# rhuangr/MARL-Maze

Measured on AMD Instinct MI355X. Metric: env-steps/sec (2-agent 10x10 maze) + PPO updates/sec, higher is better.
Workload: dtype f32; 1 GPU; PPO rollout+GAE+update over 65536 parallel 10x10 2-agent mazes per GPU (configs[2], the north-star workload: 65,536 parallel 10x10 mazes per GPU); mazes_per_gpu=65536, maze=10x10 (layout 19x19), horizon=16, global_batch=1048575, minibatch=209715, minibatch_steps_per_iter=25, parallelism=dp1, rollout=stream launches, gemm=x2, parity_mode=True

## Files before the change

### include/marlmaze.h

```cpp
#ifndef MARLMAZE_H
#define MARLMAZE_H

#include <stdint.h>

#ifdef __cplusplus
extern "C" {
#endif

#define MM_OBS_DIM 65
#define MM_MASK_DIM 6
#define MM_RNG_WORDS 625
#define MM_MAX_SIDE 41
#define MM_MAZES_PER_BLOCK 32

#define MM_E_ARG (-1)
#define MM_E_SIZE (-2)

#define MM_ST_GEN_FAIL 1u
#define MM_ST_BAD_MOVE 2u

typedef struct {
    int8_t x, y, dir, flags;
    int8_t lmx, lmy, olsx, olsy;
    int8_t minx, maxx, miny, maxy;
// ... 149 lines not shown
              const uint16_t* w1, const float* b1, int N1, const uint16_t* w2, const float* b2, int N2, float* out,
              int ldc, void* stream);
int mm_trunk3_head_sample_ok(int prec, int M, int K0, int N0, int N1, int N2, int lda);
int mm_trunk3_head_sample(int prec, const float* h0, int lda, int M, int K0, const uint16_t* w0, const float* b0,
                          int N0, const uint16_t* w1, const float* b1, int N1, const uint16_t* w2, const float* b2,
                          int N2, const float* head_w, const float* head_b, const uint8_t* masks, uint64_t seed,
                          uint64_t offset, const uint64_t* offset_dev, int8_t* actions, float* logp,
                          float* joint_logp, float* logits, float* h3, int ldh3, void* stream);

int mm_ppo_loss_partials(int M);
int mm_ppo_loss(const float* heads, const uint8_t* masks, const int8_t* actions, const float* old_logp,
                const float* adv, int M, float clip, float* coef, float* partial, void* stream);
int mm_ppo_loss_bwd(const float* heads, const uint8_t* masks, const int8_t* actions, const float* coef,
                    const float* dloss, int M, float* dheads, void* stream);

int mm_colsum(const float* x, long R, int N, float* part, int G, float* out, void* stream);
typedef struct {
    const float* x;
    long R;
    int N;
    float* out;
} mm_colsum_seg_t;
typedef struct {
    const float* x;
    long n;
    int S;
    float* out;
} mm_wsum_seg_t;
long mm_colsum_multi_ws_len(const mm_colsum_seg_t* segs, int nseg);
int mm_colsum_multi(const mm_colsum_seg_t* segs, int nseg, float* ws, void* stream);
// ... 136 lines not shown
```

### marl-maze_amd/csrc/policy_device.h

```cpp
#pragma once
#include <hip/hip_runtime.h>
#include <math.h>
#include <stdint.h>

#include "marlmaze.h"

namespace mm {

__device__ __forceinline__ uint4 philox(uint4 c, uint2 k) {
#pragma unroll
    for (int r = 0; r < 10; r++) {
        const uint32_t lo0 = 0xD2511F53u * c.x, hi0 = __umulhi(0xD2511F53u, c.x);
        const uint32_t lo1 = 0xCD9E8D57u * c.z, hi1 = __umulhi(0xCD9E8D57u, c.z);
        c = make_uint4(hi1 ^ c.y ^ k.x, lo1, hi0 ^ c.w ^ k.y, lo0);
        k.x += 0x9E3779B9u;
        k.y += 0xBB67AE85u;
    }
    return c;
}

__device__ __forceinline__ float u01(uint32_t x) { return (float)(x >> 8) * (1.0f / 16777216.0f); }

template <int MODE>
__device__ __forceinline__ float act_row(const float ml[5], float kl, const uint8_t* __restrict__ mk, int row,
// ... 98 lines not shown
        if constexpr (MODE == MM_ACT_SAMPLE) offset += offset_dev ? *offset_dev : 0ull;
        lp = act_row<MODE>(l, kl, masks + (size_t)row * MM_MASK_DIM, row, seed, offset, move, mark);
        act[2 * row] = (int8_t)move;
        act[2 * row + 1] = (int8_t)mark;
        if (logp) logp[row] = lp;
        if (logits) {
#pragma unroll
            for (int o = 0; o < 5; o++) logits[(size_t)row * 6 + o] = l[o];
            logits[(size_t)row * 6 + 5] = kl;
        }
    }
    const float other = __shfl_down(lp, kHeadLanes);
    if (joint && lead && (row & 1) == 0) joint[row >> 1] = lp + (row + 1 < M ? other : 0.f);
}

}
```

### marl-maze_amd/csrc/rl_kernels.hip

```cpp
#include <hip/hip_runtime.h>
#include <math.h>
#include <stdint.h>

#include <algorithm>

#include "marlmaze.h"
#include "policy_device.h"

namespace mm {

struct GaeArgs {
    const float* rew;
    const float* val;
    const uint8_t* done;
    const float* lv;
    int T, N;
    float g, gl;
    float* adv;
    float* rtg;
};

__device__ __forceinline__ float gae_delta(float r, float v, bool d, bool have_next, float v_next, bool d_next,
                                           float g) {
    if (d || !have_next) return __fsub_rn(r, v);
// ... 230 lines not shown
                                    __uint_as_float(v[3]));
            }
        }
#pragma unroll
        for (int s = 0; s < NS; s++) heads_fma4(hv[s], W + 4 * j + 32 * s, kSpan, acc);
    } else if (row < M) {
        heads_row_dot(h + (size_t)row * ldh, K, W, kSpan, j, acc);
    }
    heads_butterfly(acc);
    float v = acc[0];
#pragma unroll
    for (int o = 1; o < 6; o++) v = j == o ? acc[o] : v;
    if (row < M && j < 6) logits[(size_t)row * 6 + j] = v + b[j];
}

__device__ __forceinline__ float row_logp(const float* z, const uint8_t* mk, int move, int mark, float* grad) {
    float mx = -INFINITY;
#pragma unroll
    for (int j = 0; j < 5; j++)
        if (mk[j]) mx = fmaxf(mx, z[j]);
    float se = 0.f;
    float e[5];
#pragma unroll
    for (int j = 0; j < 5; j++) {
        e[j] = mk[j] ? expf(z[j] - mx) : 0.f;
        se += e[j];
    }
    const float lse = logf(se);
    const float lpm = mk[move] ? (z[move] - mx) - lse : -INFINITY;
    const float k = mk[5] ? z[5] : -INFINITY;
    const float p = 1.f / (1.f + expf(-k));
    const float pm = mark ? p : 1.f - p;
    if (grad) {
        const float inv = 1.f / se;
#pragma unroll
        for (int j = 0; j < 5; j++) grad[j] = mk[j] ? ((j == move ? 1.f : 0.f) - e[j] * inv) : 0.f;
        grad[5] = mk[5] ? (mark ? 1.f - p : -p) : 0.f;
    }
    return lpm + logf(pm);
}

constexpr int kLossThreads = 256;

__global__ __launch_bounds__(kLossThreads) void k_ppo_loss(const float* __restrict__ z, const uint8_t* __restrict__ mk,
                                                           const int8_t* __restrict__ act,
                                                           const float* __restrict__ old_lp,
                                                           const float* __restrict__ adv, int M, float clip,
                                                           float* __restrict__ coef, float* __restrict__ partial) {
    __shared__ float red[kLossThreads];
    const int i = blockIdx.x * kLossThreads + threadIdx.x;
    float term = 0.f;
    if (i < M) {
        float lp = 0.f;
#pragma unroll
        for (int a = 0; a < 2; a++) {
            const int r = 2 * i + a;
            lp += row_logp(z + (size_t)r * 6, mk + (size_t)r * 6, act[2 * r], act[2 * r + 1], nullptr);
        }
        const float ratio = expf(lp - old_lp[i]);
        const float A = adv[i];
        const float s1 = ratio * A;
        const float rc = fminf(fmaxf(ratio, 1.f - clip), 1.f + clip);
        const float s2 = rc * A;
        term = fminf(s1, s2);
        const bool inside = ratio >= 1.f - clip && ratio <= 1.f + clip;
        float dd;
        if (s1 < s2) dd = A;
        else if (s1 > s2) dd = inside ? A : 0.f;
        else dd = 0.5f * A + (inside ? 0.5f * A : 0.f);
        coef[i] = -dd * ratio / (float)M;
    }
    red[threadIdx.x] = term;
    __syncthreads();
    for (int w = kLossThreads / 2; w > 0; w >>= 1) {
        if (threadIdx.x < w) red[threadIdx.x] += red[threadIdx.x + w];
        __syncthreads();
    }
    if (threadIdx.x == 0) partial[blockIdx.x] = red[0];
}

__global__ __launch_bounds__(256) void k_ppo_loss_bwd(const float* __restrict__ z, const uint8_t* __restrict__ mk,
                                                      const int8_t* __restrict__ act, const float* __restrict__ coef,
                                                      const float* __restrict__ dloss, int M,
                                                      float* __restrict__ dz) {
    const int r = blockIdx.x * blockDim.x + threadIdx.x;
    if (r >= 2 * M) return;
    float g[6];
    row_logp(z + (size_t)r * 6, mk + (size_t)r * 6, act[2 * r], act[2 * r + 1], g);
    const float c = coef[r >> 1] * dloss[0];
#pragma unroll
    for (int j = 0; j < 6; j++) dz[(size_t)r * 6 + j] = c * g[j];
}
// ... 258 lines not shown
```

### marl-maze_amd/csrc/x3mlp.hip

```cpp
#include <hip/hip_runtime.h>
#include <stdint.h>
#include <stdlib.h>

#include <algorithm>
#include <type_traits>

#include "marlmaze.h"
#include "policy_device.h"

namespace mm {
namespace x3 {

typedef __attribute__((ext_vector_type(8))) short bf16x8;
typedef __attribute__((ext_vector_type(4))) float f32x4;
typedef __attribute__((ext_vector_type(8))) _Float16 f16x8;

enum { P_X3 = MM_PREC_X3, P_F16 = MM_PREC_F16, P_X2 = MM_PREC_X2 };
template <int P>
struct Prec {
    static constexpr int kPlanes = P == P_X3 ? 3 : P == P_X2 ? 2 : 1;
    static constexpr int kBlk = 512 * kPlanes;
    static constexpr bool kScaled = P != P_X3;
};
constexpr float kX2Lo = 2048.f;
// ... 1803 lines not shown
            const int row = 16 * tn + 4 * (lane >> 4) + g;
            if (row < N && col < K) out[(size_t)row * K + col] = v[g] * cscale;
        }
    };
#pragma unroll
    for (int r = 0; r < RN; r++)
#pragma unroll
        for (int tk = 0; tk < NTK; tk++) put(acc[r * NTK + tk], RN * wave + r, tk);
#pragma unroll
    for (int e = 0; e < EX; e++) {
        const int j = wave + kWgWaves * e;
        if (j < kRem) put(acc[RN * NTK + e], kWgWaves * RN + j / NTK, j % NTK);
    }
}

constexpr int tr_pitch(int T) {
    int w = 4 * T;
    while (w % 16 != 4) w++;
    return w;
}

template <int TN, int NTK>
__global__ __launch_bounds__(kWgThreads) void k_wgrad_tr(const uint32_t* __restrict__ dy, int lddy,
                                                         const uint32_t* __restrict__ x, int ldx, int M, int N, int K,
                                                         int rows, int nslices, int ncb, float cscale,
                                                         float* __restrict__ ws) {
    constexpr int P = P_X2;
    constexpr int RN = TN / kWgWaves;
    constexpr int kRem = (TN - kWgWaves * RN) * NTK;
    constexpr int EX = (kRem + kWgWaves - 1) / kWgWaves;
// ... 1722 lines not shown
}

extern "C" int mm_gemm_wgrad_slices(int prec, int M, int N, int K) {
    if (M <= 0 || N <= 0 || K <= 0 || (prec != MM_PREC_X3 && prec != MM_PREC_F16 && prec != MM_PREC_X2))
        return MM_E_ARG;
    const WgPlan p = wg_plan(prec, M, N, K);
    return p.TPW ? p.nslices : MM_E_ARG;
}

extern "C" int mm_gemm_wgrad_partials(int prec, const float* dy, int lddy, float dscale, const float* x, int ldx, int M,
                                      int N, int K, float cscale, float* ws, void* stream) {
    if (M <= 0) return MM_E_ARG;
    return gemm_wgrad(prec, dy, lddy, dscale, x, ldx, M, N, K, cscale, ws, nullptr, stream);
}

extern "C" int mm_critic_update_ok(int M, int K0, int ldx) {
    if (M <= 0 || K0 <= 128 || K0 > 132 || (K0 & 1) || (ldx & 1) || ldx < K0) return 0;
    const size_t wmax = std::max(ldx, 64);
    if ((size_t)(M + 320) * wmax * 4 >= ((size_t)1 << 31)) return 0;
    if (!bres_enabled()) return 0;
    BresPlan pl;
    int cfg = C_PAIR;
    return bres_plan(MM_PREC_X2, M, 64, K0, ldx, 64, true, pl, cfg) && bres_plan(MM_PREC_X2, M, 64, 64, 64, 64, true, pl, cfg) &&
                   bres_plan(MM_PREC_X2, M, 1, 64, 64, 1, false, pl, cfg)
               ? 1
               : 0;
}

extern "C" int mm_critic_update(const float* x, int ldx, int K0, int M, const float* rtg, const uint16_t* w0_tp,
                                const float* b0, const uint16_t* w1_tp, const uint16_t* w1t_tp, const float* b1,
// ... 25 lines not shown
```

### marl-maze_amd/marlmaze/PPO.py

```python
import math
import os
import random
import warnings

import numpy as np
import torch

from . import _lib, networks, ops, rollout, update, x3
from .dist import DP
from .networks import Actor, Critic

MODEL_PATH = "PPO.pth"
CRITIC_STREAM = os.environ.get("MARLMAZE_CRITIC_STREAM", "on")
CRITIC_STREAM_MAX_SAMPLES = int(os.environ.get("MARLMAZE_CRITIC_STREAM_MAX", "65536"))


def _ppo_loss_fwd(heads, mk, a8, old_logp, adv, clip):
    L = _lib.lib()
    M = old_logp.shape[0]
    old_logp, adv = old_logp.contiguous(), adv.contiguous()
    coef = torch.empty(M, dtype=torch.float32, device=heads.device)
    part = torch.empty(L.mm_ppo_loss_partials(M), dtype=torch.float32, device=heads.device)
    _lib.check(L.mm_ppo_loss(_lib.ptr(heads), _lib.ptr(mk), _lib.ptr(a8), _lib.ptr(old_logp), _lib.ptr(adv), M,
                             float(clip), _lib.ptr(coef), _lib.ptr(part), _lib.stream_ptr()), "mm_ppo_loss")
# ... 164 lines not shown
        mk = _u8(masks)
        if out is None:
            out = torch.empty(2, dtype=torch.float32, device=obs.device)
        beside = CRITIC_STREAM == "on" or (CRITIC_STREAM == "auto" and M <= CRITIC_STREAM_MAX_SAMPLES)
        with x3.cached_packs():
            x3.pack_many(self.critic.pack_specs() + self.actor.pack_specs())
            with _lib.on_side(_lib.side_stream("critic", obs.device) if beside else None) as critic_side:
                xc = obs.reshape(M, -1)
                if self.critic.fused_update_ok(xc):
                    _, mse_part = self.critic.train_update_fused(xc, rtg)
                else:
                    V, csaved = self.critic.train_forward(xc)
                    mse_part, dv = update.mse_loss(V, rtg)
                    with x3.deferred():
                        self.critic.train_backward(csaved, dv)
            heads, asaved = self.actor.train_forward(obs.reshape(2 * M, 65))
            coef, ppo_part = _ppo_loss_fwd(heads, mk, a8, old_logp, adv, self.clip)
            dz = _ppo_loss_bwd(heads, mk, a8, coef, self._one)
            with x3.deferred():
                self.actor.train_backward(asaved, dz)
            critic_side.join(mse_part)
            update.losses_final(ppo_part, mse_part, M, out)
        return out[0], out[1]

    def _minibatch_grads_host(self, obs, act, old_logp, adv, rtg, masks):
        V = self.critic(obs).view(-1)
        cur = self.policy_logp(obs, act, masks)
        ratio = torch.exp(cur - old_logp)
        s1 = ratio * adv
        s2 = torch.clamp(ratio, 1 - self.clip, 1 + self.clip) * adv
        actor_loss = -torch.mean(torch.min(s1, s2))
        critic_loss = torch.nn.functional.mse_loss(V, rtg)
        self.actor_optim.zero_grad(set_to_none=True)
        self.critic_optim.zero_grad(set_to_none=True)
        (actor_loss + critic_loss).backward()
# ... 225 lines not shown
```

### marl-maze_amd/marlmaze/_lib.py

```python
import ctypes
import os

import torch

PKG_ROOT = os.path.dirname(os.path.dirname(os.path.abspath(__file__)))
LIB_PATH = os.environ.get("MARLMAZE_LIB") or os.path.join(PKG_ROOT, "libmarlmaze.so")

OBS_DIM = 65
MASK_DIM = 6
RNG_WORDS = 625
MAX_SIDE = 41
MAZES_PER_BLOCK = 32

ST_GEN_FAIL = 1
ST_BAD_MOVE = 2

GAE_AUTO, GAE_COLUMN, GAE_WALK, GAE_SCAN = 0, 1, 2, 3

ACT_SAMPLE, ACT_GREEDY = 0, 1
ACT_MODES = {"sample": ACT_SAMPLE, "greedy": ACT_GREEDY}

EVAL_WORDS = 32
EV_EPISODES, EV_SOLVED, EV_TIMEOUTS, EV_SUM_LEN, EV_SUM_LEN_SOLVED, EV_SUM_SHORT_SOLVED = 0, 1, 2, 3, 4, 5
EV_MIN_LEN_SOLVED, EV_MAX_LEN_SOLVED, EV_SUM_RATIO_Q16, EV_BAD_SHORT = 6, 7, 8, 9
# ... 24 lines not shown
           "mm_actor_front_grad_len", "mm_actor_front_partial_len", "mm_actor_front_bwd", "mm_actor_front_bwd_ex",
           "mm_actor_front_bwd_to", "mm_actor_front_bwd_grid",
           "mm_x3_tp_len", "mm_x3_tp_pack", "mm_x3_nt", "mm_x3_nt_f32a", "mm_x3_mbits_len",
           "mm_x3_heads_bwd", "mm_ppo_loss_partials", "mm_ppo_loss", "mm_ppo_loss_bwd",
           "mm_gemm_tp_len", "mm_gemm_tp_pack", "mm_gemm_nt", "mm_gemm_nt_algo", "mm_gemm_wgrad_algo", "mm_gemm_wgrad_ws_len",
           "mm_gemm_wgrad", "mm_colsum", "mm_mse_loss_partials", "mm_mse_loss", "mm_losses_final",
           "mm_clip_adam_ws_len", "mm_clip_adam", "mm_gemm_tp_pack_multi", "mm_gemm_wgrad_slices",
           "mm_gemm_wgrad_partials", "mm_colsum_multi_ws_len", "mm_colsum_multi", "mm_wsum_multi", "mm_critic_value",
           "mm_gemm_range_flag", "mm_gemm_nt_h", "mm_gemm_a16_ok", "mm_gemm_wgrad_h", "mm_gemm_wgrad_partials_h",
           "mm_heads_fwd_h16", "mm_x3_heads_bwd_h16", "mm_trunk3_ok", "mm_trunk3",
           "mm_trunk3_head_sample_ok", "mm_trunk3_head_sample", "mm_actor_front_fwd_h16",
           "mm_actor_front_fwd_h16_ex", "mm_head_act", "mm_act", "mm_eval_init", "mm_eval_accum",
           "mm_env_dist", "mm_env_par", "mm_par_init", "mm_par_accum",
           "mm_elog_state_words", "mm_elog_init", "mm_elog_start", "mm_elog_step",
           "mm_gemm_x2p_ok", "mm_x3_heads_bwd_x2p",
           "mm_critic_update_ok", "mm_critic_update")
VERSION = 308

PREC_X3, PREC_F16, PREC_X2 = 0, 1, 2
FRONT_BWD = {"mfma": 0, "valu": 1}
FRONT_FWD = {"row1": 0, "row2": 1, "mfma": 2}
GEMM_ALGO = {"auto": 0, "stream": 1}
GEMM_A_F16, GEMM_C_F16, GEMM_B_F16 = 1, 2, 4
GEMM_A_X2P, GEMM_C_X2P, GEMM_B_X2P = 8, 16, 32


class EnvDesc(ctypes.Structure):
    _fields_ = [
        ("n", ctypes.c_int32), ("size_w", ctypes.c_int32), ("size_h", ctypes.c_int32),
        ("max_timestep", ctypes.c_int32), ("difficulty", ctypes.c_int32),
        ("rand_start", ctypes.c_int32), ("rand_sizes", ctypes.c_int32),
# ... 178 lines not shown
                                             P]),
                           ("mm_x3_heads_bwd_h16", [P, i32, P, P, i32, i32, P, P, f32, P]),
                           ("mm_gemm_a16_ok", [i32, i32, i32, i32, i32]),
                           ("mm_gemm_wgrad_h", [i32, i32, P, i32, f32, P, i32, i32, i32, i32, f32, P, P, P]),
                           ("mm_gemm_wgrad_partials_h", [i32, i32, P, i32, f32, P, i32, i32, i32, i32, f32, P, P]),
                           ("mm_heads_fwd_h16", [P, i32, i32, P, P, i32, P, P]),
                           ("mm_trunk3_ok", [i32, i32, i32, i32, i32, i32, i32]),
                           ("mm_trunk3", [i32, P, i32, i32, i32, P, P, i32, P, P, i32, P, P, i32, P, i32, P]),
                           ("mm_trunk3_head_sample_ok", [i32, i32, i32, i32, i32, i32, i32]),
                           ("mm_actor_front_fwd_h16", [P, P, i32, i32, i32, P, P]),
                           ("mm_actor_front_fwd_h16_ex", [P, P, i32, i32, i32, P, i32, P]),
                           ("mm_gemm_x2p_ok", [i32, i32, i32]),
                           ("mm_x3_heads_bwd_x2p", [P, i32, P, P, i32, i32, P, P, f32, P]),
                           ("mm_critic_update_ok", [i32, i32, i32]),
                           ("mm_critic_update", [P, i32, i32, i32] + [P] * 18),
                           ("mm_trunk3_head_sample", [i32, P, i32, i32, i32, P, P, i32, P, P, i32, P, P, i32, P, P, P,
                                                      u64, u64, P, P, P, P, P, P, i32, P])):
            if hasattr(L, name):
                getattr(L, name).argtypes = args
                getattr(L, name).restype = i32
        L.mm_colsum_multi_ws_len.argtypes = [ctypes.POINTER(ColsumSeg), i32]
        L.mm_colsum_multi_ws_len.restype = ctypes.c_long
        L.mm_colsum_multi.argtypes = [ctypes.POINTER(ColsumSeg), i32, P, P]
        L.mm_colsum_multi.restype = i32
        L.mm_wsum_multi.argtypes = [ctypes.POINTER(WsumSeg), i32, P]
        L.mm_wsum_multi.restype = i32
        L.mm_x3_mbits_len.argtypes = [i32]
        L.mm_x3_mbits_len.restype = ctypes.c_long
        L.mm_x3_nt_f32a.restype = i32
        L.mm_actor_front_ws_len.restype = i32
# ... 71 lines not shown
```

### marl-maze_amd/marlmaze/networks.py

```python
import ctypes
import math
import os

import numpy as np
import torch
import torch.nn as nn
import torch.nn.functional as F

FEATURE_DIMS = [4, 4, 4, 4, 4, 4, 4, 4, 4, 4, 4, 4, 2, 2, 1, 4, 1, 1, 1, 1, 1, 1, 2]
FEATURE_AMOUNT = len(FEATURE_DIMS)
OBS_SPACE = int(np.sum(FEATURE_DIMS))
EMBEDDING_DIM = 20
KQ_DIM = 10
_SQRT_KQ = float(np.sqrt(KQ_DIM))


class Projection(nn.Module):

    def __init__(self, parity_mode=True):
        super().__init__()
        self.layers = nn.ModuleList([nn.Linear(d, EMBEDDING_DIM) for d in FEATURE_DIMS])
        self.parity_mode = parity_mode
        starts = np.zeros(FEATURE_AMOUNT, np.int64) if parity_mode else np.cumsum([0] + FEATURE_DIMS[:-1])
        self.register_buffer("_starts", torch.as_tensor(starts), persistent=False)
# ... 130 lines not shown
    s = _grad_scale(dy.shape[0], prec)
    if x3.is_planes(dy):
        return x3.wgrad(dy, x, prec=prec, dscale=1.0, cscale=1.0 / s, out=out, nk=nk)
    if dy.dtype == torch.float16:
        return x3.wgrad(dy.contiguous(), x, prec=prec, dscale=1.0, cscale=1.0 / s, out=out)
    return x3.wgrad(dy.contiguous(), x, prec=prec, dscale=s, out=out)


F16_ACT = os.environ.get("MARLMAZE_F16_ACT", "1") != "0"
F16_H0 = os.environ.get("MARLMAZE_F16_H0", "1") != "0"


X2_PLANES = os.environ.get("MARLMAZE_X2_PLANES", "1") != "0"

CRITIC_FUSED = os.environ.get("MARLMAZE_CRITIC_FUSED", "1") != "0"


class _SavedPlanes(torch.Tensor):

    _STORAGE = ("as_subclass",)

    @staticmethod
    def __new__(cls, p):
        return torch.Tensor._make_subclass(cls, p)

    def planes(self):
        return self.as_subclass(torch.Tensor)

    def values(self):
        p = self.planes()
# ... 104 lines not shown
        _lib.check(_lib.lib().mm_heads_fwd_h16(_lib.ptr(h), K, K, _lib.ptr(wh), _lib.ptr(bh), M, _lib.ptr(out),
                                                _lib.stream_ptr()), "mm_heads_fwd_h16")
        return out
    if wh.shape[0] != 6 or K % 4 or K > 1024:
        return x3.gemm(h, x3.pack(wh, prec="x3"), bias=bh)
    h, wh, bh = h.contiguous(), wh.contiguous(), bh.contiguous()
    out = torch.empty((M, 6), dtype=torch.float32, device=h.device)
    step = max(1, (2 ** 31 - 1) // (4 * K))
    for r0 in range(0, M, step):
        m = min(step, M - r0)
        _lib.check(_lib.lib().mm_heads_fwd(_lib.ptr(h[r0:r0 + m]), K, K, _lib.ptr(wh), _lib.ptr(bh), m,
                                            _lib.ptr(out[r0:r0 + m]), _lib.stream_ptr()), "mm_heads_fwd")
    return out


def _heads_bwd(dz, h, wh, bits, out_w=None, out_b=None, oscale=None, x2p=False):
    from . import x3

    dwh = _wgrad(dz, h, "x3", out=out_w)
    dbh = x3.colsum(dz, out=out_b)
    dy, cs = x3.heads_bwd(dz, wh, bits, oscale=oscale, x2p=x2p)
    return dy, cs, dwh, dbh


class _EngineTrunk(torch.autograd.Function):

    @staticmethod
    def forward(ctx, prec, h0, *params):
        hs, bits = _mlp_fwd(h0, params[0::2], params[1::2], prec, True)
        ctx.save_for_backward(*hs, *params[0::2])
        ctx.bits, ctx.prec = bits, prec
        return hs[-1]

    @staticmethod
# ... 190 lines not shown
        return ok

    def _mlp(self, h):
        if self._engine(h):
            params = self._mlp_params()
            if torch.is_grad_enabled() and (h.requires_grad or any(p.requires_grad for p in params)):
                return _EngineTrunk.apply(self.gemm_prec, h, *params)
            with torch.no_grad():
                hs, _ = _mlp_fwd(h, params[0::2], params[1::2], self.gemm_prec, False)
            return hs[-1]
        act = self.activation()
        for lin in self.layers:
            h = act(F.linear(h, lin.weight, lin.bias))
        return h

    def train_forward(self, x):
        x = x.contiguous()
        params = self._mlp_params()
        wl = [lin.weight for lin in self.layers]
        act16 = (_act16(self.gemm_prec, x.shape[0], [w_.shape[0] for w_ in wl],
                        [(w_.shape[0], w_.shape[1]) for w_ in wl[1:]]) and (wl[-1].shape[0] + 31) // 32 == 9)
        h16 = act16 and F16_H0 and wl[0].shape[1] % 4 == 0
        ws, h0 = _front_fwd(x, self.projection.parity_mode, front_params(self.projection, self.attention), h16=h16)
        if not self._engine(h0):
            raise ValueError("Actor.train_forward needs the GPU engine's shapes (ReLU, widths <= 272)")
        x2p = len(wl) > 1 and _x2p(self.gemm_prec, x.shape[0], [tuple(w_.shape) for w_ in wl[1:]])
        hs, bits = _mlp_fwd(h0, params[0::2], params[1::2], self.gemm_prec, True, act16=act16, x2p=x2p)
        w, b = self.heads()
        z = _heads_fwd(hs[-1], w, b)
        if x2p:
            from . import x3

            hs = [_SavedPlanes(h) if x3.is_planes(h) else h for h in hs]
        return z, (x, ws, hs, bits)

    def train_backward(self, saved, dz):
        x, ws, hs, bits = saved
        hs = [h.planes() if isinstance(h, _SavedPlanes) else h for h in hs]
        L = len(self.layers)
        w, _ = self.heads()
        gw = self._adjacent(_grad_of(self.move_head.weight), _grad_of(self.mark_head.weight))
        gb = self._adjacent(_grad_of(self.move_head.bias), _grad_of(self.mark_head.bias))
        params = self._mlp_params()
        g16 = _g16(self.gemm_prec, hs, params[0::2], True)
        from . import x3

        x2p = x3.is_planes(hs[L - 1])
        dy, cs, dwh, dbh = _heads_bwd(dz.contiguous(), hs[L], w, bits[L - 1], out_w=gw, out_b=gb,
                                      oscale=_grad_scale(dz.shape[0], self.gemm_prec) if g16 or x2p else None,
                                      x2p=x2p)
        if gw is None:
            self.move_head.weight.grad.copy_(dwh[:5])
            self.mark_head.weight.grad.copy_(dwh[5:])
        if gb is None:
            self.move_head.bias.grad.copy_(dbh[:5])
            self.mark_head.bias.grad.copy_(dbh[5:])
        params = self._mlp_params()
        dh0, _ = _mlp_bwd(bits, hs, params[0::2], dy, cs, self.gemm_prec, True,
                          outs=[_grad_of(p) for p in params])
        _front_bwd_to(ws, x, self.projection.parity_mode, dh0,
                      [_grad_of(p) for p in front_params(self.projection, self.attention)])


def _front_fwd_algo(B):
    if FRONT_FWD_ALGO == "auto":
# ... 182 lines not shown
```

### marl-maze_amd/marlmaze/x3.py

```python
import weakref

import torch

from . import _lib


PRECS = {"x3": _lib.PREC_X3, "f16": _lib.PREC_F16, "x2": _lib.PREC_X2}


class TP:
    __slots__ = ("buf", "R", "C", "prec", "src")

    def __init__(self, R, C, device, buf=None, prec="x3"):
        self.R, self.C, self.prec = int(R), int(C), prec
        self.src = None
        n = _lib.lib().mm_gemm_tp_len(PRECS[prec], self.R, self.C)
        self.buf = buf if buf is not None else torch.empty(n, dtype=torch.int16, device=device)
        assert self.buf.numel() >= n

    def ptr(self):
        return _lib.ptr(self.buf)


_PACK_CACHE = {}
# ... 316 lines not shown
                _lib.ptr(ws), _lib.stream_ptr())
        _lib.check(L.mm_gemm_wgrad_partials_h(PRECS[prec], flags, *args) if flags
                   else L.mm_gemm_wgrad_partials(PRECS[prec], *args), "mm_gemm_wgrad_partials")
        d = _DEFER[-1]
        d.sums.append(_lib.WsumSeg(_lib.ptr(ws), N * K, S, _lib.ptr(out)))
        d.keep += [ws, out]
        return out
    ws = torch.empty(max(1, L.mm_gemm_wgrad_ws_len(M, N, K)), dtype=torch.float32, device=dy.device)
    args = (_lib.ptr(dy), _pitch(dy), float(dscale), _lib.ptr(x), _pitch(x), M, N, K, cs,
            _lib.ptr(ws), _lib.ptr(out), _lib.stream_ptr())
    _lib.check(L.mm_gemm_wgrad_h(PRECS[prec], flags, *args) if flags else L.mm_gemm_wgrad(PRECS[prec], *args),
               "mm_gemm_wgrad")
    return out


def mbits(M, device):
    return torch.empty(_lib.lib().mm_x3_mbits_len(int(M)), dtype=torch.int32, device=device)


def nt(a, b, bias=None, relu=False, mask=None, out=None, out_tp=None, want_f32=True, mbits_in=None,
       mbits_out=None, colsum=None):
    N, K = b.R, b.C
    if isinstance(a, TP):
        assert a.C == K, (a.C, K)
        M, dev = a.R, a.buf.device
    else:
        assert a.dtype == torch.float32 and a.dim() == 2 and a.stride(1) == 1 and a.shape[1] == K, (a.shape, K)
        M, dev = a.shape[0], a.device
    if want_f32 and out is None:
        out = torch.empty((M, N), dtype=torch.float32, device=dev)
# ... 71 lines not shown
```

Measured before the change: 7.704 million env-steps/s.

## Fuse actor heads forward, PPO loss, dz and head weight-grad into one pipelined kernel

Adds a k_heads_pass kernel that streams the last hidden activation through LDS with a triple-buffered DMA pipeline. In one pass it computes the 6 head logits, the per-row log-prob, the PPO clipped loss coefficient and term, dz, and per-slice head weight-gradient partials using x3-split MFMA. This replaces the separate heads forward, ppo_loss, ppo_loss_bwd and head wgrad passes, avoiding repeated reads of the [2M,264] activation and several kernel launches. It is enabled by default through MARLMAZE_HEADS_FUSED, adds a small partial-reduction kernel, and uses a complex wave-specialized schedule with hand-written waitcnt values that carries correctness risk.

```diff
diff --git a/include/marlmaze.h b/include/marlmaze.h
--- a/include/marlmaze.h
+++ b/include/marlmaze.h
@@ -187,6 +187,12 @@
 int mm_ppo_loss_bwd(const float* heads, const uint8_t* masks, const int8_t* actions, const float* coef,
                     const float* dloss, int M, float* dheads, void* stream);
 
+int mm_heads_pass_ok(int M, int K, int ldh);
+int mm_heads_pass(const float* h, int ldh, int K, const float* w, const float* b, const uint8_t* masks,
+                  const int8_t* actions, const float* old_logp, const float* adv, const float* dloss, int M,
+                  float clip, float* logits, float* coef, float* term, float* partial, float* dz, float* ws,
+                  void* stream);
+
 int mm_colsum(const float* x, long R, int N, float* part, int G, float* out, void* stream);
 typedef struct {
     const float* x;
diff --git a/marl-maze_amd/csrc/policy_device.h b/marl-maze_amd/csrc/policy_device.h
--- a/marl-maze_amd/csrc/policy_device.h
+++ b/marl-maze_amd/csrc/policy_device.h
@@ -136,4 +136,54 @@
     if (joint && lead && (row & 1) == 0) joint[row >> 1] = lp + (row + 1 < M ? other : 0.f);
 }
 
+__device__ __forceinline__ float row_logp(const float* z, const uint8_t* mk, int move, int mark, float* grad) {
+    float mx = -INFINITY;
+#pragma unroll
+    for (int j = 0; j < 5; j++)
+        if (mk[j]) mx = fmaxf(mx, z[j]);
+    float se = 0.f;
+    float e[5];
+#pragma unroll
+    for (int j = 0; j < 5; j++) {
+        e[j] = mk[j] ? expf(z[j] - mx) : 0.f;
+        se += e[j];
+    }
+    const float lse = logf(se);
+    const float lpm = mk[move] ? (z[move] - mx) - lse : -INFINITY;
+    const float k = mk[5] ? z[5] : -INFINITY;
+    const float p = 1.f / (1.f + expf(-k));
+    const float pm = mark ? p : 1.f - p;
+    if (grad) {
+        const float inv = 1.f / se;
+#pragma unroll
+        for (int j = 0; j < 5; j++) grad[j] = mk[j] ? ((j == move ? 1.f : 0.f) - e[j] * inv) : 0.f;
+        grad[5] = mk[5] ? (mark ? 1.f - p : -p) : 0.f;
+    }
+    return lpm + logf(pm);
 }
+
+__device__ __forceinline__ float ppo_sample(float lp, float old_lp, float A, float clip, int M, float& term) {
+    const float ratio = expf(lp - old_lp);
+    const float s1 = ratio * A;
+    const float rc = fminf(fmaxf(ratio, 1.f - clip), 1.f + clip);
+    const float s2 = rc * A;
+    term = fminf(s1, s2);
+    const bool inside = ratio >= 1.f - clip && ratio <= 1.f + clip;
+    float dd;
+    if (s1 < s2) dd = A;
+    else if (s1 > s2) dd = inside ? A : 0.f;
+    else dd = 0.5f * A + (inside ? 0.5f * A : 0.f);
+    return -dd * ratio / (float)M;
+}
+
+constexpr int kLossThreads = 256;
+__device__ __forceinline__ void ppo_tree256(float term, float* red) {
+    red[threadIdx.x] = term;
+    __syncthreads();
+    for (int w = kLossThreads / 2; w > 0; w >>= 1) {
+        if (threadIdx.x < w) red[threadIdx.x] += red[threadIdx.x + w];
+        __syncthreads();
+    }
+}
+
+}
diff --git a/marl-maze_amd/csrc/rl_kernels.hip b/marl-maze_amd/csrc/rl_kernels.hip
--- a/marl-maze_amd/csrc/rl_kernels.hip
+++ b/marl-maze_amd/csrc/rl_kernels.hip
@@ -268,33 +268,6 @@
     if (row < M && j < 6) logits[(size_t)row * 6 + j] = v + b[j];
 }
 
-__device__ __forceinline__ float row_logp(const float* z, const uint8_t* mk, int move, int mark, float* grad) {
-    float mx = -INFINITY;
-#pragma unroll
-    for (int j = 0; j < 5; j++)
-        if (mk[j]) mx = fmaxf(mx, z[j]);
-    float se = 0.f;
-    float e[5];
-#pragma unroll
-    for (int j = 0; j < 5; j++) {
-        e[j] = mk[j] ? expf(z[j] - mx) : 0.f;
-        se += e[j];
-    }
-    const float lse = logf(se);
-    const float lpm = mk[move] ? (z[move] - mx) - lse : -INFINITY;
-    const float k = mk[5] ? z[5] : -INFINITY;
-    const float p = 1.f / (1.f + expf(-k));
-    const float pm = mark ? p : 1.f - p;
-    if (grad) {
-        const float inv = 1.f / se;
-#pragma unroll
-        for (int j = 0; j < 5; j++) grad[j] = mk[j] ? ((j == move ? 1.f : 0.f) - e[j] * inv) : 0.f;
-        grad[5] = mk[5] ? (mark ? 1.f - p : -p) : 0.f;
-    }
-    return lpm + logf(pm);
-}
-
-constexpr int kLossThreads = 256;
 
 __global__ __launch_bounds__(kLossThreads) void k_ppo_loss(const float* __restrict__ z, const uint8_t* __restrict__ mk,
                                                            const int8_t* __restrict__ act,
@@ -311,25 +284,9 @@
             const int r = 2 * i + a;
             lp += row_logp(z + (size_t)r * 6, mk + (size_t)r * 6, act[2 * r], act[2 * r + 1], nullptr);
         }
-        const float ratio = expf(lp - old_lp[i]);
-        const float A = adv[i];
-        const float s1 = ratio * A;
-        const float rc = fminf(fmaxf(ratio, 1.f - clip), 1.f + clip);
-        const float s2 = rc * A;
-        term = fminf(s1, s2);
-        const bool inside = ratio >= 1.f - clip && ratio <= 1.f + clip;
-        float dd;
-        if (s1 < s2) dd = A;
-        else if (s1 > s2) dd = inside ? A : 0.f;
-        else dd = 0.5f * A + (inside ? 0.5f * A : 0.f);
-        coef[i] = -dd * ratio / (float)M;
-    }
-    red[threadIdx.x] = term;
-    __syncthreads();
-    for (int w = kLossThreads / 2; w > 0; w >>= 1) {
-        if (threadIdx.x < w) red[threadIdx.x] += red[threadIdx.x + w];
-        __syncthreads();
-    }
+        coef[i] = ppo_sample(lp, old_lp[i], adv[i], clip, M, term);
+    }
+    ppo_tree256(term, red);
     if (threadIdx.x == 0) partial[blockIdx.x] = red[0];
 }
 
diff --git a/marl-maze_amd/csrc/x3mlp.hip b/marl-maze_amd/csrc/x3mlp.hip
--- a/marl-maze_amd/csrc/x3mlp.hip
+++ b/marl-maze_amd/csrc/x3mlp.hip
@@ -1841,6 +1841,284 @@
     }
 }
 
+constexpr int kHpK = 264, kHpTiles = 17, kHpPitchW = 288;
+constexpr int kHpStage = 32 * kHpK;
+constexpr int kHpIns = kHpStage * 4 / 1024;
+constexpr int kHpDmaWaves = 3, kHpDmaW0 = 4, kHpLossWave = 7;
+constexpr int kHpInsW = kHpIns / kHpDmaWaves;
+static_assert(kHpIns * 1024 == kHpStage * 4 && kHpInsW * kHpDmaWaves == kHpIns, "whole DMA instructions");
+
+struct HpArgs {
+    const float* h;
+    const float* w;
+    const float* b;
+    const uint8_t* masks;
+    const int8_t* act;
+    const float* old_lp;
+    const float* adv;
+    const float* dloss;
+    int M;
+    float clip;
+    int rows, nslices;
+    float* logits;
+    float* coef;
+    float* term;
+    float* dz;
+    float* ws;
+};
+
+__global__ __launch_bounds__(kWgThreads) void k_heads_pass(HpArgs ha) {
+    __shared__ __attribute__((aligned(16))) float raw0[kHpStage];
+    __shared__ __attribute__((aligned(16))) float raw1[kHpStage];
+    __shared__ __attribute__((aligned(16))) float raw2[kHpStage];
+    __shared__ __attribute__((aligned(16))) float Wl[6 * kHpPitchW];
+    __shared__ __attribute__((aligned(16))) float zl[2][32 * 6];
+    __shared__ __attribute__((aligned(16))) float dzl[2][32 * 6];
+    __shared__ __attribute__((aligned(16))) uint8_t mkl[32 * 8];
+    const int lane = threadIdx.x & 63;
+    const int wave = __builtin_amdgcn_readfirstlane(threadIdx.x >> 6);
+    const int s = blockIdx.x;
+    if (s >= ha.nslices) return;
+    const int R = 2 * ha.M;
+    const int m_begin = s * ha.rows, nrows = min(R, m_begin + ha.rows) - m_begin;
+    const int nsteps = (nrows + 31) / 32;
+    __amdgpu_buffer_rsrc_t rs = __builtin_amdgcn_make_buffer_rsrc((void*)(ha.h + (size_t)m_begin * kHpK), (short)0,
+                                                                  (int)(nrows * kHpK * 4), 0x00020000);
+    asm volatile("" : "+s"(rs));
+    const bool dma_wave = wave >= kHpDmaW0 && wave < kHpDmaW0 + kHpDmaWaves;
+    uint32_t ob[3][kHpInsW];
+#pragma unroll
+    for (int k = 0; k < kHpInsW; k++) {
+        const int i = (wave - kHpDmaW0) + kHpDmaWaves * k;
+#pragma unroll
+        for (int t = 0; t < 3; t++) {
+            ob[t][k] = (uint32_t)(t * kHpStage * 4 + 1024 * i + 16 * lane);
+            asm volatile("" : "+v"(ob[t][k]));
+        }
+    }
+    const uint32_t step3 = 3u * kHpStage * 4u;
+    auto issue = [&](auto tc, int st) {
+        constexpr int T = decltype(tc)::value;
+        const uint32_t base = lds_addr(T == 0 ? raw0 : T == 1 ? raw1 : raw2);
+        __builtin_amdgcn_sched_barrier(0);
+#pragma unroll
+        for (int k = 0; k < kHpInsW; k++) {
+            const int i = (wave - kHpDmaW0) + kHpDmaWaves * k;
+            if (st >= 3) asm volatile("v_add_u32 %0, %0, %1" : "+v"(ob[T][k]) : "s"(step3));
+            dma16(rs, ob[T][k], base + 1024u * (uint32_t)i);
+        }
+        __builtin_amdgcn_sched_barrier(0);
+    };
+    auto wait_dma = [&](bool later_in_flight) {
+        asm volatile("" ::: "memory");
+        __builtin_amdgcn_sched_barrier(0);
+        if (later_in_flight) __builtin_amdgcn_s_waitcnt(0x0F70 | (kHpInsW & 15) | ((kHpInsW >> 4) << 14));
+        else __builtin_amdgcn_s_waitcnt(0x0F70);
+        __builtin_amdgcn_sched_barrier(0);
+        asm volatile("" ::: "memory");
+    };
+    auto barrier = [&]() {
+        __builtin_amdgcn_sched_barrier(0);
+        __builtin_amdgcn_s_waitcnt((15 << 0) | (7 << 4) | (0 << 8) | (3 << 14));
+        __builtin_amdgcn_s_barrier();
+        asm volatile("" ::: "memory");
+        __builtin_amdgcn_sched_barrier(0);
+    };
+
+    struct RowIn {
+        uint32_t m01, m23, m45, a01;
+        float old, adv;
+    };
+    auto load_rows = [&](int st) {
+        RowIn in{0u, 0u, 0u, 0u, 0.f, 0.f};
+        const int gr = m_begin + 32 * st + (lane & 31);
+        if (32 * st + (lane & 31) < nrows) {
+            const uint16_t* mp = reinterpret_cast<const uint16_t*>(ha.masks + (size_t)gr * MM_MASK_DIM);
+            in.m01 = mp[0];
+            in.m23 = mp[1];
+            in.m45 = mp[2];
+            in.a01 = reinterpret_cast<const uint16_t*>(ha.act)[gr];
+            in.old = ha.old_lp[gr >> 1];
+            in.adv = ha.adv[gr >> 1];
+        }
+        return in;
+    };
+
+    for (int e = threadIdx.x; e < 6 * kHpPitchW; e += kWgThreads) {
+        const int o = e / kHpPitchW, c = e - o * kHpPitchW;
+        Wl[e] = c < kHpK ? ha.w[o * kHpK + c] : 0.f;
+    }
+    const int hj = threadIdx.x & (kHeadLanes - 1), hrow = (threadIdx.x >> 3) & 31;
+    const float bj = hj < 6 ? ha.b[hj] : 0.f;
+    const float dloss0 = ha.dloss[0];
+    RowIn ring[3];
+    ring[0] = load_rows(0);
+    ring[1] = ring[2] = ring[0];
+    constexpr std::integral_constant<int, 0> c0{};
+    constexpr std::integral_constant<int, 1> c1{};
+    constexpr std::integral_constant<int, 2> c2{};
+    if (dma_wave) {
+        issue(c0, 0);
+        if (nsteps > 1) issue(c1, 1);
+        wait_dma(nsteps > 1);
+    }
+    barrier();
+
+    constexpr int kHpMaxT = 4;
+    const int ntile = wave < 4 ? (wave == 0 ? 2 : 1) : (wave < kHpLossWave ? 4 : 0);
+    auto tile_of = [&](int e) { return wave < 4 ? (e == 0 ? wave : 16) : 4 * (wave - 3) + e; };
+    f32x4 acc[kHpMaxT], accx;
+#pragma unroll
+    for (int u = 0; u < kHpMaxT; u++) acc[u] = f32x4{0.f, 0.f, 0.f, 0.f};
+    accx = acc[0];
+    bf16x8 bq[2][kHpMaxT][3];
+    auto bfrag_step = [&](auto pc, const float* stage) {
+        constexpr int PAR = decltype(pc)::value;
+        const int n = lane & 15, c = lane >> 4;
+#pragma unroll
+        for (int e = 0; e < kHpMaxT; e++) {
+            if (e < ntile) {
+                const int col = 16 * tile_of(e) + n;
+                const float* src = stage + 8 * c * kHpK + (col < kHpK ? col : kHpK - 1);
+                float v[8];
+#pragma unroll
+                for (int i = 0; i < 8; i++) v[i] = src[i * kHpK];
+                uint32_t h[4], m[4], l[4];
+#pragma unroll
+                for (int k = 0; k < 4; k++) split2(v[2 * k], v[2 * k + 1], h[k], m[k], l[k]);
+                bq[PAR][e][0] = __builtin_bit_cast(bf16x8, make_uint4(h[0], h[1], h[2], h[3]));
+                bq[PAR][e][1] = __builtin_bit_cast(bf16x8, make_uint4(m[0], m[1], m[2], m[3]));
+                bq[PAR][e][2] = __builtin_bit_cast(bf16x8, make_uint4(l[0], l[1], l[2], l[3]));
+            }
+        }
+    };
+    auto mfma_step = [&](auto pc, const float* dzs) {
+        constexpr int PAR = decltype(pc)::value;
+        float v[8];
+        const int n = lane & 15, c = lane >> 4;
+#pragma unroll
+        for (int i = 0; i < 8; i++) v[i] = n < 6 ? dzs[(8 * c + i) * 6 + n] : 0.f;
+        uint32_t h[4], m[4], l[4];
+#pragma unroll
+        for (int k = 0; k < 4; k++) split2(v[2 * k], v[2 * k + 1], h[k], m[k], l[k]);
+        bf16x8 a[3];
+        a[0] = __builtin_bit_cast(bf16x8, make_uint4(h[0], h[1], h[2], h[3]));
+        a[1] = __builtin_bit_cast(bf16x8, make_uint4(m[0], m[1], m[2], m[3]));
+        a[2] = __builtin_bit_cast(bf16x8, make_uint4(l[0], l[1], l[2], l[3]));
+#pragma unroll
+        for (int e = 0; e < kHpMaxT; e++)
+            if (e < ntile) acc[e] = mma<P_X3>(a, bq[PAR][e], acc[e], accx);
+    };
+    auto heads_step = [&](const float* stage, float* zs, int st) {
+        const float* hr = stage + hrow * kHpK;
+        float a6[6] = {0.f, 0.f, 0.f, 0.f, 0.f, 0.f};
+        float4 hv[9];
+#pragma unroll
+        for (int q = 0; q < 9; q++) {
+            const int c = 4 * hj + 32 * q;
+            hv[q] = make_float4(0.f, 0.f, 0.f, 0.f);
+            if (c < kHpK) hv[q] = *reinterpret_cast<const float4*>(hr + c);
+        }
+#pragma unroll
+        for (int q = 0; q < 9; q++) heads_fma4(hv[q], Wl + 4 * hj + 32 * q, kHpPitchW, a6);
+        heads_butterfly(a6);
+        float v = a6[0];
+#pragma unroll
+        for (int o = 1; o < 6; o++) v = hj == o ? a6[o] : v;
+        if (hj < 6) {
+            const float z = v + bj;
+            zs[hrow * 6 + hj] = z;
+            if (32 * st + hrow < nrows) ha.logits[(size_t)(m_begin + 32 * st + hrow) * 6 + hj] = z;
+        }
+    };
+    auto loss_step = [&](const RowIn& in, const float* zs, float* dzs, int st) {
+        const int r = lane & 31;
+        const bool valid = 32 * st + r < nrows;
+        uint16_t* mw = reinterpret_cast<uint16_t*>(mkl + r * 8);
+        mw[0] = (uint16_t)in.m01;
+        mw[1] = (uint16_t)in.m23;
+        mw[2] = (uint16_t)in.m45;
+        float g[6];
+        const float lpr = row_logp(zs + r * 6, mkl + r * 8, (int)(int8_t)(in.a01 & 0xFFu), (int)(int8_t)(in.a01 >> 8), g);
+        const float other = __shfl_xor(lpr, 1);
+        float lp = 0.f;
+        lp += (lane & 1) ? other : lpr;
+        lp += (lane & 1) ? lpr : other;
+        float term;
+        const float cf = ppo_sample(lp, in.old, in.adv, ha.clip, ha.M, term);
+        const float c = cf * dloss0;
+        const int gr = m_begin + 32 * st + r;
+        const bool st_ok = valid && lane < 32;
+        if (st_ok && (lane & 1) == 0) {
+            ha.coef[gr >> 1] = cf;
+            ha.term[gr >> 1] = term;
+        }
+#pragma unroll
+        for (int j = 0; j < 6; j++) {
+            const float d = c * g[j];
+            dzs[r * 6 + j] = valid ? d : 0.f;
+            if (st_ok) ha.dz[(size_t)gr * 6 + j] = d;
+        }
+    };
+    auto phase = [&](auto pc6, int p) {
+        constexpr int P6 = decltype(pc6)::value;
+        constexpr std::integral_constant<int, P6 % 3> ct{};
+        constexpr std::integral_constant<int, (P6 + 2) % 3> ct2{};
+        constexpr std::integral_constant<int, P6 & 1> cp{};
+        const float* stage = P6 % 3 == 0 ? raw0 : P6 % 3 == 1 ? raw1 : raw2;
+        (void)ct;
+        if (dma_wave && p + 2 < nsteps) issue(ct2, p + 2);
+        if (p >= 2) mfma_step(cp, dzl[P6 & 1]);
+        if (p < nsteps) bfrag_step(cp, stage);
+        if (wave < 4) {
+            if (p < nsteps) heads_step(stage, zl[P6 & 1], p);
+        } else if (wave == kHpLossWave) {
+            if (p + 1 < nsteps) ring[(P6 + 1) % 3] = load_rows(p + 1);
+            if (p >= 1 && p <= nsteps) loss_step(ring[(P6 + 2) % 3], zl[1 - (P6 & 1)], dzl[1 - (P6 & 1)], p - 1);
+        }
+        if (dma_wave && p + 1 < nsteps) wait_dma(p + 2 < nsteps);
+        barrier();
+    };
+    constexpr std::integral_constant<int, 3> c3{};
+    constexpr std::integral_constant<int, 4> c4{};
+    constexpr std::integral_constant<int, 5> c5{};
+    const int nph = nsteps + 2;
+    for (int p = 0; p < nph; p += 6) {
+        phase(c0, p);
+        if (p + 1 < nph) phase(c1, p + 1);
+        if (p + 2 < nph) phase(c2, p + 2);
+        if (p + 3 < nph) phase(c3, p + 3);
+        if (p + 4 < nph) phase(c4, p + 4);
+        if (p + 5 < nph) phase(c5, p + 5);
+    }
+#pragma unroll
+    for (int t = 0; t < 3; t++)
+#pragma unroll
+        for (int k = 0; k < kHpInsW; k++) asm volatile("" ::"v"(ob[t][k]));
+    asm volatile("" ::"s"(rs), "s"(step3));
+    float* out = ha.ws + (size_t)s * 6 * kHpK;
+#pragma unroll
+    for (int e = 0; e < kHpMaxT; e++) {
+        const int tk = tile_of(e);
+        if (e < ntile) {
+            const int col = 16 * tk + (lane & 15);
+#pragma unroll
+            for (int g = 0; g < 4; g++) {
+                const int row = 4 * (lane >> 4) + g;
+                if (row < 6 && col < kHpK) out[(size_t)row * kHpK + col] = acc[e][g];
+            }
+        }
+    }
+}
+
+__global__ __launch_bounds__(kLossThreads) void k_ppo_partials(const float* __restrict__ term, int M,
+                                                               float* __restrict__ partial) {
+    __shared__ float red[kLossThreads];
+    const int i = blockIdx.x * kLossThreads + threadIdx.x;
+    ppo_tree256(i < M ? term[i] : 0.f, red);
+    if (threadIdx.x == 0) partial[blockIdx.x] = red[0];
+}
+
 constexpr int tr_pitch(int T) {
     int w = 4 * T;
     while (w % 16 != 4) w++;
@@ -3593,6 +3871,30 @@
     return gemm_wgrad(prec, dy, lddy, dscale, x, ldx, M, N, K, cscale, ws, nullptr, stream);
 }
 
+extern "C" int mm_heads_pass_ok(int M, int K, int ldh) {
+    if (M <= 0 || K != kHpK || ldh != kHpK) return 0;
+    if ((size_t)2 * M * kHpK * 4 >= ((size_t)1 << 31)) return 0;
+    const WgPlan p = wg_plan(MM_PREC_X3, 2 * M, 6, kHpK);
+    return p.TN == 1 && p.NTK == kHpTiles && p.ncb == 1 && p.rows % 32 == 0 ? 1 : 0;
+}
+
+extern "C" int mm_heads_pass(const float* h, int ldh, int K, const float* w, const float* b, const uint8_t* masks,
+                             const int8_t* actions, const float* old_logp, const float* adv, const float* dloss, int M,
+                             float clip, float* logits, float* coef, float* term, float* partial, float* dz, float* ws,
+                             void* stream) {
+    if (!h || !w || !b || !masks || !actions || !old_logp || !adv || !dloss || !logits || !coef || !term || !partial ||
+        !dz || !ws || ((uintptr_t)h & 15))
+        return MM_E_ARG;
+    if (mm_heads_pass_ok(M, K, ldh) != 1) return MM_E_ARG;
+    const WgPlan p = wg_plan(MM_PREC_X3, 2 * M, 6, kHpK);
+    hipStream_t s = (hipStream_t)stream;
+    HpArgs ha{h, w, b, masks, actions, old_logp, adv, dloss, M, clip, p.rows, p.nslices, logits, coef, term, dz, ws};
+    hipLaunchKernelGGL(k_heads_pass, dim3(p.nslices), dim3(kWgThreads), 0, s, ha);
+    hipLaunchKernelGGL(k_ppo_partials, dim3((M + mm::kLossThreads - 1) / mm::kLossThreads), dim3(mm::kLossThreads), 0,
+                       s, term, M, partial);
+    return (int)hipGetLastError();
+}
+
 extern "C" int mm_critic_update_ok(int M, int K0, int ldx) {
     if (M <= 0 || K0 <= 128 || K0 > 132 || (K0 & 1) || (ldx & 1) || ldx < K0) return 0;
     const size_t wmax = std::max(ldx, 64);
diff --git a/marl-maze_amd/marlmaze/PPO.py b/marl-maze_amd/marlmaze/PPO.py
--- a/marl-maze_amd/marlmaze/PPO.py
+++ b/marl-maze_amd/marlmaze/PPO.py
@@ -202,11 +202,16 @@
                     mse_part, dv = update.mse_loss(V, rtg)
                     with x3.deferred():
                         self.critic.train_backward(csaved, dv)
-            heads, asaved = self.actor.train_forward(obs.reshape(2 * M, 65))
-            coef, ppo_part = _ppo_loss_fwd(heads, mk, a8, old_logp, adv, self.clip)
-            dz = _ppo_loss_bwd(heads, mk, a8, coef, self._one)
+            fused = self.actor.train_forward_loss(obs.reshape(2 * M, 65), mk, a8, old_logp, adv, self.clip, self._one)
+            if fused is not None:
+                heads, coef, ppo_part, dz, asaved, wpart = fused
+            else:
+                wpart = None
+                heads, asaved = self.actor.train_forward(obs.reshape(2 * M, 65))
+                coef, ppo_part = _ppo_loss_fwd(heads, mk, a8, old_logp, adv, self.clip)
+                dz = _ppo_loss_bwd(heads, mk, a8, coef, self._one)
             with x3.deferred():
-                self.actor.train_backward(asaved, dz)
+                self.actor.train_backward(asaved, dz, heads_partials=wpart)
             critic_side.join(mse_part)
             update.losses_final(ppo_part, mse_part, M, out)
         return out[0], out[1]
diff --git a/marl-maze_amd/marlmaze/_lib.py b/marl-maze_amd/marlmaze/_lib.py
--- a/marl-maze_amd/marlmaze/_lib.py
+++ b/marl-maze_amd/marlmaze/_lib.py
@@ -62,7 +62,7 @@
            "mm_env_dist", "mm_env_par", "mm_par_init", "mm_par_accum",
            "mm_elog_state_words", "mm_elog_init", "mm_elog_start", "mm_elog_step",
            "mm_gemm_x2p_ok", "mm_x3_heads_bwd_x2p",
-           "mm_critic_update_ok", "mm_critic_update")
+           "mm_critic_update_ok", "mm_critic_update", "mm_heads_pass_ok", "mm_heads_pass")
 VERSION = 308
 
 PREC_X3, PREC_F16, PREC_X2 = 0, 1, 2
@@ -271,6 +271,8 @@
                            ("mm_x3_heads_bwd_x2p", [P, i32, P, P, i32, i32, P, P, f32, P]),
                            ("mm_critic_update_ok", [i32, i32, i32]),
                            ("mm_critic_update", [P, i32, i32, i32] + [P] * 18),
+                           ("mm_heads_pass_ok", [i32, i32, i32]),
+                           ("mm_heads_pass", [P, i32, i32] + [P] * 7 + [i32, f32] + [P] * 7),
                            ("mm_trunk3_head_sample", [i32, P, i32, i32, i32, P, P, i32, P, P, i32, P, P, i32, P, P, P,
                                                       u64, u64, P, P, P, P, P, P, i32, P])):
             if hasattr(L, name):
diff --git a/marl-maze_amd/marlmaze/networks.py b/marl-maze_amd/marlmaze/networks.py
--- a/marl-maze_amd/marlmaze/networks.py
+++ b/marl-maze_amd/marlmaze/networks.py
@@ -168,6 +168,8 @@
 X2_PLANES = os.environ.get("MARLMAZE_X2_PLANES", "1") != "0"
 
 CRITIC_FUSED = os.environ.get("MARLMAZE_CRITIC_FUSED", "1") != "0"
+
+HEADS_FUSED = os.environ.get("MARLMAZE_HEADS_FUSED", "1") != "0"
 
 
 class _SavedPlanes(torch.Tensor):
@@ -302,10 +304,15 @@
     return out
 
 
-def _heads_bwd(dz, h, wh, bits, out_w=None, out_b=None, oscale=None, x2p=False):
-    from . import x3
-
-    dwh = _wgrad(dz, h, "x3", out=out_w)
+def _heads_bwd(dz, h, wh, bits, out_w=None, out_b=None, oscale=None, x2p=False, w_partials=None):
+    from . import x3
+
+    if w_partials is not None:
+        if out_w is None:
+            out_w = torch.empty(tuple(wh.shape), dtype=torch.float32, device=dz.device)
+        dwh = x3.wsum(w_partials[0], w_partials[1], out_w)
+    else:
+        dwh = _wgrad(dz, h, "x3", out=out_w)
     dbh = x3.colsum(dz, out=out_b)
     dy, cs = x3.heads_bwd(dz, wh, bits, oscale=oscale, x2p=x2p)
     return dy, cs, dwh, dbh
@@ -526,7 +533,7 @@
             h = act(F.linear(h, lin.weight, lin.bias))
         return h
 
-    def train_forward(self, x):
+    def _train_trunk(self, x):
         x = x.contiguous()
         params = self._mlp_params()
         wl = [lin.weight for lin in self.layers]
@@ -538,15 +545,33 @@
             raise ValueError("Actor.train_forward needs the GPU engine's shapes (ReLU, widths <= 272)")
         x2p = len(wl) > 1 and _x2p(self.gemm_prec, x.shape[0], [tuple(w_.shape) for w_ in wl[1:]])
         hs, bits = _mlp_fwd(h0, params[0::2], params[1::2], self.gemm_prec, True, act16=act16, x2p=x2p)
-        w, b = self.heads()
-        z = _heads_fwd(hs[-1], w, b)
+        h_last = hs[-1]
         if x2p:
             from . import x3
 
             hs = [_SavedPlanes(h) if x3.is_planes(h) else h for h in hs]
-        return z, (x, ws, hs, bits)
-
-    def train_backward(self, saved, dz):
+        return (x, ws, hs, bits), h_last
+
+    def train_forward(self, x):
+        saved, h_last = self._train_trunk(x)
+        w, b = self.heads()
+        return _heads_fwd(h_last, w, b), saved
+
+    def train_forward_loss(self, x, mk, a8, old_logp, adv, clip, dloss):
+        from . import _lib, x3
+
+        w, b = self.heads()
+        K = self.layers[-1].weight.shape[0]
+        if (not HEADS_FUSED or self.gemm_prec == "f16" or w.shape[0] != 6 or x.shape[0] % 2
+                or not _lib.lib().mm_heads_pass_ok(x.shape[0] // 2, K, K)):
+            return None
+        saved, h_last = self._train_trunk(x)
+        if not x3.heads_pass_ok(h_last, w.shape[0]):
+            raise ValueError("Actor.train_forward_loss: the last hidden activation is not fp32 [2M, 264] contiguous")
+        z, coef, part, dz, partials = x3.heads_pass(h_last, w, b, mk, a8, old_logp, adv, dloss, clip)
+        return z, coef, part, dz, saved, partials
+
+    def train_backward(self, saved, dz, heads_partials=None):
         x, ws, hs, bits = saved
         hs = [h.planes() if isinstance(h, _SavedPlanes) else h for h in hs]
         L = len(self.layers)
@@ -560,7 +585,7 @@
         x2p = x3.is_planes(hs[L - 1])
         dy, cs, dwh, dbh = _heads_bwd(dz.contiguous(), hs[L], w, bits[L - 1], out_w=gw, out_b=gb,
                                       oscale=_grad_scale(dz.shape[0], self.gemm_prec) if g16 or x2p else None,
-                                      x2p=x2p)
+                                      x2p=x2p, w_partials=heads_partials)
         if gw is None:
             self.move_head.weight.grad.copy_(dwh[:5])
             self.mark_head.weight.grad.copy_(dwh[5:])
diff --git a/marl-maze_amd/marlmaze/x3.py b/marl-maze_amd/marlmaze/x3.py
--- a/marl-maze_amd/marlmaze/x3.py
+++ b/marl-maze_amd/marlmaze/x3.py
@@ -354,6 +354,48 @@
     return out
 
 
+def wsum(ws, S, out):
+    assert out.is_contiguous() and ws.numel() == S * out.numel()
+    seg = _lib.WsumSeg(_lib.ptr(ws), out.numel(), int(S), _lib.ptr(out))
+    if _DEFER:
+        d = _DEFER[-1]
+        d.sums.append(seg)
+        d.keep += [ws, out]
+        return out
+    arr = (_lib.WsumSeg * 1)(seg)
+    _lib.check(_lib.lib().mm_wsum_multi(arr, 1, _lib.stream_ptr()), "mm_wsum_multi")
+    return out
+
+
+def heads_pass_ok(h, n_heads):
+    if (h is None or is_planes(h) or h.dtype != torch.float32 or h.dim() != 2 or not h.is_contiguous()
+            or n_heads != 6 or h.shape[0] % 2 or h.data_ptr() % 16):
+        return False
+    return bool(_lib.lib().mm_heads_pass_ok(h.shape[0] // 2, h.shape[1], h.stride(0)))
+
+
+def heads_pass(h, wh, bh, mk, a8, old_logp, adv, dloss, clip):
+    L = _lib.lib()
+    R, K = h.shape
+    M, dev = R // 2, h.device
+    f32 = dict(dtype=torch.float32, device=dev)
+    z, dz = torch.empty((R, 6), **f32), torch.empty((R, 6), **f32)
+    coef, term = torch.empty(M, **f32), torch.empty(M, **f32)
+    part = torch.empty(L.mm_ppo_loss_partials(M), **f32)
+    S = L.mm_gemm_wgrad_slices(PRECS["x3"], R, 6, K)
+    _lib.check(S if S < 0 else 0, "mm_gemm_wgrad_slices")
+    ws = torch.empty(S * 6 * K, **f32)
+    wh, bh, old_logp, adv = wh.contiguous(), bh.contiguous(), old_logp.contiguous(), adv.contiguous()
+    assert mk.dtype == torch.uint8 and mk.is_contiguous() and mk.numel() == R * 6
+    assert a8.dtype == torch.int8 and a8.is_contiguous() and a8.numel() == R * 2
+    assert old_logp.dtype == adv.dtype == torch.float32 and old_logp.numel() == adv.numel() == M
+    _lib.check(L.mm_heads_pass(_lib.ptr(h), h.stride(0), K, _lib.ptr(wh), _lib.ptr(bh), _lib.ptr(mk), _lib.ptr(a8),
+                               _lib.ptr(old_logp), _lib.ptr(adv), _lib.ptr(dloss), M, float(clip), _lib.ptr(z),
+                               _lib.ptr(coef), _lib.ptr(term), _lib.ptr(part), _lib.ptr(dz), _lib.ptr(ws),
+                               _lib.stream_ptr()), "mm_heads_pass")
+    return z, coef, part, dz, (ws, S)
+
+
 def mbits(M, device):
     return torch.empty(_lib.lib().mm_x3_mbits_len(int(M)), dtype=torch.int32, device=device)
 
```

Result: no change. 7.758 million env-steps/s (median of 5 runs) (+0.7%).
